# JKc66/CircuitVision

Measured on AMD Instinct MI355X. Metric: circuit images/sec (YOLOv11 640² + SAM2.1-L 1024²) at 1/2/4/8 MI355X, higher is better.
Workload: dtype f16; 1 GPU; YOLO11-n 640x640 batch=32 f16 forward+decode+NMS (BASELINE configs[1]) + SAM2.1 Hiera-L 1024x1024 2 x batch=16 f16 learned-prompt wrapper forward (configs[2]) on the same images, per GPU and step; nc=62, weights=seeded random (SAM: LoRA merged), streams=3

## Files before the change

circuitvision_amd/_lib.py:

```python
import ctypes as C
import os

_HERE = os.path.dirname(os.path.abspath(__file__))
LIB_PATH = os.environ.get("CVMI_LIB_PATH") or os.path.join(_HERE, "libcvmi355.so")

F16, F32, BF16 = 0, 1, 2
ACT_NONE, ACT_SILU, ACT_RELU, ACT_GELU, ACT_SIGMOID = 0, 1, 2, 3, 4


class CvmiError(RuntimeError):
    pass


class ConvDesc(C.Structure):
    _fields_ = [
        ("x0", C.c_void_p), ("x1", C.c_void_p), ("w", C.c_void_p), ("bias", C.c_void_p),
        ("res", C.c_void_p), ("y", C.c_void_p),
        ("x0_ld", C.c_int), ("x1_ld", C.c_int), ("res_ld", C.c_int), ("y_ld", C.c_int),
        ("c0", C.c_int), ("c1", C.c_int), ("up0", C.c_int), ("up1", C.c_int),
        ("B", C.c_int), ("H", C.c_int), ("W", C.c_int), ("OH", C.c_int), ("OW", C.c_int),
        ("KH", C.c_int), ("KW", C.c_int), ("stride", C.c_int), ("pad", C.c_int),
        ("N", C.c_int), ("Kpad", C.c_int), ("act", C.c_int), ("dtype", C.c_int),
        ("out_f32", C.c_int), ("scalar_gather", C.c_int),
        ("res_mod", C.c_int), ("act_after_res", C.c_int), ("shuffle_cout", C.c_int), ("res_rep", C.c_int),
        ("row_stats", C.c_void_p),
    ]


class C3k2Desc(C.Structure):
    _fields_ = [
        ("x", C.c_void_p), ("y", C.c_void_p),
        ("w0", C.c_void_p), ("w1", C.c_void_p), ("w2", C.c_void_p), ("w3", C.c_void_p),
        ("b0", C.c_void_p), ("b1", C.c_void_p), ("b2", C.c_void_p), ("b3", C.c_void_p),
        ("x_ld", C.c_int), ("y_ld", C.c_int), ("kpad0", C.c_int), ("kpad1", C.c_int), ("kpad2", C.c_int), ("kpad3", C.c_int),
        ("B", C.c_int), ("H", C.c_int), ("W", C.c_int), ("c1", C.c_int), ("c", C.c_int), ("h", C.c_int), ("c2", C.c_int),
        ("fuse_cv1", C.c_int), ("shortcut", C.c_int), ("dtype", C.c_int),
    ]


class DwPwDesc(C.Structure):
    _fields_ = [
        ("x", C.c_void_p), ("y", C.c_void_p), ("wd", C.c_void_p), ("bd", C.c_void_p),
        ("w1", C.c_void_p), ("b1", C.c_void_p), ("w2", C.c_void_p), ("b2", C.c_void_p),
        ("x_ld", C.c_int), ("y_ld", C.c_int), ("kpad1", C.c_int), ("kpad2", C.c_int),
        ("B", C.c_int), ("H", C.c_int), ("W", C.c_int), ("C", C.c_int), ("N1", C.c_int), ("N2", C.c_int),
        ("dtype", C.c_int),
    ]


class AttnDesc(C.Structure):
    _fields_ = [
        ("q", C.c_void_p), ("k", C.c_void_p), ("v", C.c_void_p), ("o", C.c_void_p),
        ("q_sb", C.c_longlong), ("q_sh", C.c_longlong), ("q_st", C.c_longlong),
        ("k_sb", C.c_longlong), ("k_sh", C.c_longlong), ("k_st", C.c_longlong),
        ("v_sb", C.c_longlong), ("v_sh", C.c_longlong), ("v_st", C.c_longlong),
        ("o_sb", C.c_longlong), ("o_sh", C.c_longlong), ("o_st", C.c_longlong),
        ("B", C.c_int), ("heads", C.c_int), ("Nq", C.c_int), ("Nk", C.c_int),
        ("dqk", C.c_int), ("dv", C.c_int), ("scale", C.c_float), ("dtype", C.c_int),
# ... 142 lines not shown
```

circuitvision_amd/csrc/igemm.hip:

```cpp
#include "conv_epilogue.hpp"

namespace {

struct ConvKArgs {
  const char* x0; const char* x1; const char* w; const float* bias; const char* res; char* y;
  int x0_ld, x1_ld, res_ld, y_ld;
  int c0, ctot;
  int up0, up1;
  int H, W, OH, OW, KW, stride, pad;
  int M, N, K, Kpad;
  int act, scalar_gather;
  int res_mod, act_after_res, shuf_c, res_rep;
  int plain;
  int rows2;
  int nb_n;
  int bias_off;
  int per_xcd;
  float* stats;
  int im2col_shift;
  FastDiv div_ctot, div_kw;
};

__device__ __attribute__((aligned(256))) unsigned char cvmi_zero_page[256];

__device__ __forceinline__ int xcd_remap(int wg, int nwg) {
  const int q = nwg >> 3, r = nwg & 7, xcd = wg & 7, j = wg >> 3;
  return (xcd < r ? xcd * (q + 1) : r * (q + 1) + (xcd - r) * q) + j;
}

#define CLEAR_ACC32(acc, NI, NJ) \
  _Pragma("unroll") for (int i = 0; i < NI; ++i) \
  _Pragma("unroll") for (int j = 0; j < NJ; ++j) \
  _Pragma("unroll") for (int r = 0; r < 16; ++r) acc[i][j][r] = 0.f
// ... 1335 lines not shown
  constexpr int glds_min_tiles = 512;
  if ((a.plain || a.rows2) && a.K % (16 / (int)sizeof(T)) == 0 && (a.Kpad * (int)sizeof(T)) % 128 == 0 && a.K * (int)sizeof(T) >= 256 &&
      ((a.K * (int)sizeof(T)) % 128 == 0 || a.K >= 256) && N >= (a.rows2 ? 64 : 96) &&
      (long long)cdiv(M, 128) * cdiv(N, 128) >= glds_min_tiles) {
    if (N <= 640) return launch_glds<T, TO, 128, 64, 2, 2>(a, stream);
    return launch_glds<T, TO, 128, 128, 2, 2>(a, stream);
  }
  if (N <= 32) {
    if (M >= 256 * 512) return launch_cfg<T, TO, 256, 32, 4, 1>(a, stream);
    return launch_cfg<T, TO, 128, 32, 4, 1>(a, stream);
  }
  if (N <= 64) {
    if (M >= 128 * 512) return launch_cfg<T, TO, 128, 64, 2, 2>(a, stream);
    return launch_cfg<T, TO, 64, 64, 2, 2>(a, stream);
  }
  if (sizeof(TO) == 4 && sizeof(T) == 2 && N <= 192) return launch_cfg<T, TO, 128, 64, 2, 2>(a, stream);
  const long long blocks128 = (long long)cdiv(M, 128) * cdiv(N, 128);
  if (blocks128 >= 512) return launch_cfg<T, TO, 128, 128, 2, 2>(a, stream);
  return launch_cfg<T, TO, 64, 128, 2, 2>(a, stream);
}

}

int cvmi_conv_tile_try(const cvmi_conv_desc* d, hipStream_t stream);
#ifndef CVMI_OPERAND_BF16
extern "C" int cvmi_conv2d_bf16(const cvmi_conv_desc* d, cvmi_stream_t stream_);
#endif

extern "C" int CVMI_ENTRY(cvmi_conv2d)(const cvmi_conv_desc* d, cvmi_stream_t stream_) {
  CVMI_CHECK(d != nullptr, "conv2d: null descriptor");
#ifndef CVMI_OPERAND_BF16
  if (d->dtype == CVMI_BF16) return cvmi_conv2d_bf16(d, stream_);
#endif
  CVMI_CHECK(d->x0 && d->w && d->bias && d->y, "conv2d: null pointer");
  CVMI_CHECK(d->dtype == CVMI_T16 || d->dtype == CVMI_F32, "conv2d: bad dtype %d", d->dtype);
  const int es = d->dtype == CVMI_T16 ? 2 : 4;
  const int vec = 16 / es;
  const int oes = (d->dtype == CVMI_F32 || d->out_f32) ? 4 : 2;
  const int ovec = 16 / oes;
  CVMI_CHECK(d->B > 0 && d->H > 0 && d->W > 0 && d->OH > 0 && d->OW > 0 && d->N > 0, "conv2d: bad shape");
  CVMI_CHECK(d->KH > 0 && d->KW > 0 && d->stride > 0 && d->pad >= 0, "conv2d: bad kernel geometry");
  CVMI_CHECK(d->c0 > 0 && d->c1 >= 0 && (d->c1 == 0 || d->x1), "conv2d: bad sources");
  CVMI_CHECK((d->OH - 1) * d->stride - d->pad + d->KH - 1 < d->H + d->pad &&
             (d->OW - 1) * d->stride - d->pad + d->KW - 1 < d->W + d->pad, "conv2d: output larger than input allows");
  const int ctot = d->c0 + d->c1;
  const long long K = (long long)d->KH * d->KW * ctot;
  CVMI_CHECK(K < 65536 && d->Kpad >= K && d->Kpad % 32 == 0 && d->Kpad <= 65536, "conv2d: K=%lld Kpad=%d unsupported", K, d->Kpad);
  if (!d->scalar_gather) {
    CVMI_CHECK(d->c0 % vec == 0 && d->c1 % vec == 0, "conv2d: channels (%d,%d) not multiples of %d", d->c0, d->c1, vec);
    CVMI_CHECK(d->x0_ld % vec == 0 && (d->c1 == 0 || d->x1_ld % vec == 0), "conv2d: source ld not 16-byte aligned");
    CVMI_CHECK(((uintptr_t)d->x0 & 15) == 0 && ((uintptr_t)d->x1 & 15) == 0, "conv2d: source not 16-byte aligned");
  }
  CVMI_CHECK(d->x0_ld >= d->c0 && (d->c1 == 0 || d->x1_ld >= d->c1), "conv2d: ld smaller than channels");
  CVMI_CHECK(d->y_ld % ovec == 0 && ((uintptr_t)d->y & 15) == 0, "conv2d: output not 16-byte aligned");
  CVMI_CHECK(d->y_ld >= d->N || d->shuffle_cout > 0, "conv2d: y_ld < N");
  CVMI_CHECK(!d->res || (d->res_ld % ovec == 0 && ((uintptr_t)d->res & 15) == 0 && (d->res_ld >= d->N || d->shuffle_cout > 0)), "conv2d: residual misaligned");
  CVMI_CHECK(((uintptr_t)d->w & 15) == 0 && ((uintptr_t)d->bias & 15) == 0, "conv2d: weights misaligned");
  CVMI_CHECK(d->up0 == 0 || (d->H % 2 == 0 && d->W % 2 == 0), "conv2d: upsampled source needs even H, W");
  CVMI_CHECK(d->up1 == 0 || (d->H % 2 == 0 && d->W % 2 == 0), "conv2d: upsampled source needs even H, W");
  const long long M = (long long)d->B * d->OH * d->OW;
  CVMI_CHECK(M < (1ll << 31), "conv2d: M too large");

  ConvKArgs a;
  a.x0 = (const char*)d->x0; a.x1 = (const char*)d->x1; a.w = (const char*)d->w; a.bias = d->bias;
  a.res = (const char*)d->res; a.y = (char*)d->y;
  a.x0_ld = d->x0_ld; a.x1_ld = d->x1_ld; a.res_ld = d->res_ld; a.y_ld = d->y_ld;
// ... 36 lines not shown
```

circuitvision_amd/engine.py:

```python
import ctypes as C
import os
import threading

import torch

from . import _lib
from ._lib import BF16, F16, F32, AttnDesc, C3k2Desc, ConvDesc

TORCH_DTYPE = {F16: torch.float16, F32: torch.float32, BF16: torch.bfloat16}
ESIZE = {F16: 2, F32: 4, BF16: 2}
DTYPE_OF = {torch.float16: F16, torch.float32: F32, torch.bfloat16: BF16}


def is16(dtype):
    return dtype in (F16, BF16)


def require_gpu():
    if not torch.cuda.is_available():
        raise _lib.CvmiError("circuitvision_amd needs an MI355X (gfx950) GPU: torch.cuda.is_available() is False; "
                             "there is no CPU fallback")
    _lib.load()


# ... 525 lines not shown
        return dict(wp=wp[:C_].clone(), bp=bias[:C_].clone(), w1=w1, b1=f1[:, C_] + f1[:, C_ + 1], w2=f2[:C_].clone(), b2=bias[C_:].clone())


def op_hiera_mlp(plan, label, pm, x, gamma, beta, eps=1e-6, stats_out=None, stats_eps=1e-6, proj=None):
    lib = _lib.load()
    if proj is not None:
        pm, ao = proj[0], _as_rows(proj[1])
    assert x.dtype == F32 and x.c == pm.C and x.c0 == 0
    rows = x.B * x.H * x.W
    assert stats_out is None or (stats_out.dtype == torch.float32 and stats_out.numel() == 2 * rows and stats_out.is_contiguous()), label
    desc, b2 = None, pm.bias.data_ptr()
    if proj is not None:
        assert ao.rows == rows and ao.C == pm.C and ao.dtype == pm.dtype, label
        desc = _lib.MlpProj(ao=ao.ptr, w_packed=pm.w.data_ptr(), bp=pm.bias.data_ptr(), ao_ld=ao.ld)
        b2 += 4 * pm.C
    args = (x.ptr, x.ld, gamma.data_ptr(), beta.data_ptr(), float(eps), None if proj is not None else pm.w.data_ptr(), b2, rows, pm.C, pm.dtype,
            stats_out.data_ptr() if stats_out is not None else None, float(stats_eps))
    plan.keep.append((pm, x, gamma, beta, stats_out, proj, desc))
    sp0, fn = plan.sptr, lib.cvmi_hiera_mlp_stats
    pdesc = C.byref(desc) if desc is not None else None

    def thunk(sp=None):
        sp = sp0 if sp is None else sp
        _lib.check(fn(*args, sp, pdesc), label)

    plan.add(label, "mlp_fused", thunk, rows * pm.C * (8 + (ESIZE[pm.dtype] if proj is not None else 0)),
             2 * rows * 2 * 4 * pm.C * pm.C + (2 * rows * pm.C * pm.C if proj is not None else 0))


def tok_linear_supported(K, dtype, rows):
    return is16(dtype) and rows % 256 == 0 and bool(_lib.load().cvmi_tok_linear_supported(K))


class PackedTokLinear:

    def __init__(self, w, b, device="cuda", dtype=F16):
        N, K = w.shape
        td = TORCH_DTYPE[dtype]
        assert K % 16 == 0
        if _lib.load().cvmi_tok_linear_format(K) == 16:
            nch, ks = (N + 31) // 32, K // 32
            b = b if b is not None else torch.zeros(N)
            wx = torch.zeros(nch * 32, K)
            wx[:N] = w
            frag = wx.view(nch, 2, 16, ks, 4, 8).permute(0, 3, 1, 4, 2, 5).reshape(nch, ks * 2 * 512)
            bias = torch.zeros(nch * 32)
            bias[:N] = b
            piece = torch.zeros(nch, 512, dtype=torch.int16)
            piece[:, :64] = bias.view(nch, 32).contiguous().view(torch.int16)
            packed = torch.cat((frag.to(td).contiguous().view(torch.int16), piece), 1).contiguous()
            assert packed.numel() * 2 == _lib.load().cvmi_tok_linear_packed_bytes(K, N)
            self.w = packed.to(device)
            self.bias = torch.zeros(4, device=device)
            self.N, self.K, self.dtype = N, K, dtype
            self.param_bytes = N * K * 2
            return
        ks1, nch = K // 16 + 1, ((N + 31) // 32 + 1) // 2 * 2
        b = b if b is not None else torch.zeros(N)
        b_hi = b.to(td).float()
        b_lo = (b - b_hi).to(td).float()
        wx = torch.zeros(nch * 32, K + 16)
        wx[:N, :K], wx[:N, K], wx[:N, K + 1] = w, b_hi, b_lo
        packed = wx.view(nch, 32, ks1, 2, 8).permute(0, 2, 3, 1, 4).contiguous()
        assert packed.numel() * 2 == _lib.load().cvmi_tok_linear_packed_bytes(K, N)
        self.w = packed.to(td).to(device)
        self.bias = torch.zeros(4, device=device)
        self.N, self.K, self.dtype = N, K, dtype
        self.param_bytes = N * K * 2


def qkv_attn_rows(heads, hd=72):
    C_ = heads * hd
    rows = []
    for h in range(heads):
        for c in range(3):
            for r in range(32):
                g, lh, e = r >> 3, (r >> 2) & 1, r & 3
                d = 32 * c + 16 * (g >> 1) + 8 * lh + 4 * (g & 1) + e
                rows.append(h * hd + d if d < hd else -1)
        rows += [C_ + h * hd + n if n < hd else 2 * C_ + h * hd + n - hd if n < 2 * hd else -1 for n in range(160)]
    return rows


def qkv_attn_supported(dim, dout, heads, ws, q_pool, dtype, nwin):
    return is16(dtype) and dim == 144 and ws == 8 and nwin % 2 == 0 and (dout, heads) == ((288, 4) if q_pool else (144, 2))


def qkv_attn16_supported(dim, dout, heads, ws, q_pool, dtype, nwin):
    return is16(dtype) and dim == 288 and ws == 4 and nwin % 8 == 0 and (dout, heads) == ((576, 8) if q_pool else (288, 4))


class PackedQkvAttn:

    def __init__(self, w, b, heads, device="cuda", dtype=F16):
        N, K = w.shape
        assert N % (3 * heads) == 0
        self.rows = qkv_attn_rows(heads, N // (3 * heads))
        idx = torch.tensor(self.rows)
        keep = (idx >= 0).float()
        b = b if b is not None else torch.zeros(N)
        pt = PackedTokLinear(w[idx.clamp(min=0)] * keep[:, None], b[idx.clamp(min=0)] * keep, device, dtype)
        self.w, self.bias = pt.w, pt.bias
        self.N, self.K, self.heads, self.dtype = N, K, heads, dtype
        self.param_bytes = pt.param_bytes


def tok_linear_stats_parts(rows, K, N):
    return int(_lib.load().cvmi_tok_linear_stats_parts(rows, K, N))


def op_tok_linear(plan, label, pt, src, dst, ln=None, act=_lib.ACT_NONE, residual=False, kind="gemm", stats_in=None, stats_out=None, stats_eps=1e-6,
                  stats_parts=0):
    lib = _lib.load()
    src, dst = _as_rows(src), _as_rows(dst)
    assert src.C == pt.K and dst.C == pt.N and src.rows == dst.rows and src.rows % 256 == 0, label
    assert (src.dtype == F32) == (ln is not None) and (dst.dtype == F32) == bool(residual), label
    assert (ln is not None or src.dtype == pt.dtype) and (residual or dst.dtype == pt.dtype), label
    cast = isinstance(ln, str)
    assert not cast or ln == "cast", label
    assert stats_in is None or (ln is not None and not cast), label
    assert stats_out is None or residual, label
    out_parts = tok_linear_stats_parts(src.rows, pt.K, pt.N) if stats_out is not None else 0
    assert stats_out is None or (stats_out.dtype == torch.float32 and stats_out.numel() == 2 * src.rows * max(out_parts, 1) and stats_out.is_contiguous()), label
    assert stats_in is None or (stats_in.dtype == torch.float32 and stats_in.numel() == 2 * src.rows * max(stats_parts, 1) and stats_in.is_contiguous()), label
    gam, bet, eps = ln if (ln is not None and not cast) else (None, None, 0.0)
    args = (src.ptr, src.ld, 2 if cast else 1 if ln is not None else 0, gam.data_ptr() if gam is not None else None, bet.data_ptr() if bet is not None else None,
            float(eps), pt.w.data_ptr(), dst.ptr, dst.ld, 1 if residual else 0, src.rows, pt.K, pt.N, act, pt.dtype,
            stats_in.data_ptr() if stats_in is not None else None, int(stats_parts), stats_out.data_ptr() if stats_out is not None else None, float(stats_eps))
    plan.keep.append((pt, src, dst, gam, bet, stats_in, stats_out))
    sp0, fn = plan.sptr, lib.cvmi_tok_linear_stats

    def thunk(sp=None):
        sp = sp0 if sp is None else sp
        _lib.check(fn(*args, sp), label)

    bytes_ = src.rows * (pt.K * ESIZE[src.dtype] + pt.N * ESIZE[dst.dtype] * (2 if residual else 1))
    plan.add(label, kind, thunk, bytes_, 2 * src.rows * pt.N * pt.K)


# ... 19 lines not shown
```

circuitvision_amd/sam2.py:

```python
import hashlib
import math
import os
import threading

import numpy as np
import torch
import torch.nn.functional as TF

from . import _lib
from ._lib import ACT_GELU, ACT_NONE, ACT_RELU, ACT_SIGMOID, BF16, F16, F32
from .engine import (ESIZE, TORCH_DTYPE, is16, Buf, PackedConv, PackedHieraMlp, PackedProjMlp, PackedQkvAttn, PackedTokLinear, Plan, Rows, hiera_mlp_supported, make_attn_desc, op_attention,
                     op_call, op_cast, op_conv, op_hiera_mlp, op_layernorm, op_maxpool2, op_tok_linear, op_tok_linear_pool, require_gpu, row_stats_supported,
                     qkv_attn16_supported, qkv_attn_supported, tok_linear_stats_parts, tok_linear_supported)

LOG2E = 1.4426950408889634
HIERA_L = dict(embed_dim=144, num_heads=2, stages=(2, 6, 36, 4), global_att_blocks=(23, 33, 43), window_spec=(8, 4, 16, 8))
HIERA_T = dict(embed_dim=96, num_heads=1, stages=(1, 2, 7, 2), global_att_blocks=(5, 7, 9), window_spec=(8, 4, 14, 7))

LORA_TARGETS_REFERENCE = (
    [f"sam_mask_decoder.transformer.layers.{l}.{a}.{p}" for l in (0, 1) for a in ("self_attn", "cross_attn_token_to_image")
     for p in ("k_proj", "q_proj", "v_proj", "out_proj")]
    + [f"sam_mask_decoder.transformer.layers.{l}.mlp.layers.{j}" for l in (0, 1) for j in (0, 1)]
    + ["sam_mask_decoder.iou_prediction_head.layers.2", "sam_mask_decoder.conv_s0", "sam_mask_decoder.conv_s1",
       "image_encoder.neck.convs.2.conv", "image_encoder.neck.convs.3.conv",
       "image_encoder.trunk.blocks.44.attn.qkv", "image_encoder.trunk.blocks.44.mlp.layers.0", "image_encoder.trunk.blocks.44.proj",
       "image_encoder.trunk.blocks.47.attn.qkv", "image_encoder.trunk.blocks.47.mlp.layers.0"]
    + [f"sam_mask_decoder.transformer.layers.{l}.cross_attn_image_to_token.{p}" for l in (0, 1) for p in ("q_proj", "k_proj", "v_proj")])


MASK_DOWN = "sam_prompt_encoder.mask_downscaling"
MASK_DOWN_PARAMS = 4684


def mask_down_tensors():
    return [(f"{MASK_DOWN}.0.weight", (4, 1, 2, 2), "w"), (f"{MASK_DOWN}.0.bias", (4,), "w"),
            (f"{MASK_DOWN}.1.weight", (4,), "gamma"), (f"{MASK_DOWN}.1.bias", (4,), "w"),
            (f"{MASK_DOWN}.3.weight", (16, 4, 2, 2), "w"), (f"{MASK_DOWN}.3.bias", (16,), "w"),
            (f"{MASK_DOWN}.4.weight", (16,), "gamma"), (f"{MASK_DOWN}.4.bias", (16,), "w"),
            (f"{MASK_DOWN}.6.weight", (256, 16, 1, 1), "w"), (f"{MASK_DOWN}.6.bias", (256,), "w")]


class SamSyntheticParams:

    def __init__(self, seed=0, lora_targets=LORA_TARGETS_REFERENCE, r=4, alpha=16, std=0.02):
        self.seed, self.targets, self.r, self.scaling, self.std, self.sd = seed, set(lora_targets), r, alpha / r, std, {}
        self.mask_sd = {}
# ... 140 lines not shown
        self.pc[key] = pc
        self.param_bytes += pc.param_bytes
        return pc

    def _linear(self, key, mod, cout, cin, tok=False, row_scale=None, fuse_heads=0):
        w, b = self.p.weight(mod, (cout, cin)), self.p.bias(mod, cout)
        if row_scale is not None:
            n, f = row_scale
            w, b = w.clone(), b.clone()
            w[:n] *= f
            b[:n] *= f
        if tok and self.use_tok and is16(self.dtype) and tok_linear_supported(cin, self.dtype, 256):
            self.tl[key] = PackedTokLinear(w, b, self.device, self.dtype)
            if fuse_heads:
                self.tl[key + "_attn"] = PackedQkvAttn(w, b, fuse_heads, self.device, self.dtype)
        return self._pack(key, _lin(w), b)

    def _norm(self, key, mod, c):
        self.ln[key] = (self.p.tensor(f"{mod}.weight", (c,), "gamma").float().to(self.device),
                        self.p.tensor(f"{mod}.bias", (c,)).float().to(self.device))

    def _trunk(self):
        h = self.hiera
        E, stages, ws = h["embed_dim"], h["stages"], h["window_spec"]
        T = "image_encoder.trunk"
        w7 = self.p.weight(f"{T}.patch_embed.proj", (E, 3, 7, 7))
        w2 = torch.zeros(E, 48, 2, 2)
        m = {k: ((0, k + 1) if k < 3 else (1, k - 3)) for k in range(7)}
        for ky in range(7):
            for kx in range(7):
                (ty, sy), (tx, sx) = m[ky], m[kx]
                w2[:, (sy * 4 + sx) * 3:(sy * 4 + sx) * 3 + 3, ty, tx] = w7[:, :, ky, kx]
        self._pack("patch_embed", w2, self.p.bias(f"{T}.patch_embed.proj", E))
        g = self.image_size // 4
        pos = TF.interpolate(self.p.tensor(f"{T}.pos_embed", (1, E, 7, 7)), size=(g, g), mode="bicubic")
        win = self.p.tensor(f"{T}.pos_embed_window", (1, E, ws[0], ws[0]))
        pos = pos + win.tile([1, 1, g // ws[0], g // ws[0]])
        self.const["pos_embed"] = pos.permute(0, 2, 3, 1).reshape(g * g, E).contiguous().float().to(self.device)
        stage_ends = [sum(stages[:i]) - 1 for i in range(1, len(stages) + 1)]
        q_pool_blocks = [x + 1 for x in stage_ends[:-1]][:3]
        self.blocks, self.stage_ends = [], stage_ends
        cur, dim, heads = 1, E, h["num_heads"]
        for i in range(sum(stages)):
            dim_out, window = dim, ws[cur - 1]
            if i in h["global_att_blocks"]:
                window = 0
            if i - 1 in stage_ends:
                dim_out, heads, cur = dim * 2, heads * 2, cur + 1
            b = f"{T}.blocks.{i}"
            self._norm(f"b{i}.norm1", f"{b}.norm1", dim)
            self._linear(f"b{i}.qkv", f"{b}.attn.qkv", 3 * dim_out, dim, tok=True,
                         row_scale=(dim_out, (dim_out // heads) ** -0.5 * LOG2E) if self.q_log2 else None,
                         fuse_heads=heads if (self.qkv_attn and qkv_attn_supported(dim, dim_out, heads, window, i in q_pool_blocks, self.dtype, 2))
                         or (self.qkv_attn16 and qkv_attn16_supported(dim, dim_out, heads, window, i in q_pool_blocks, self.dtype, 8)) else 0)
            self._linear(f"b{i}.proj", f"{b}.attn.proj", dim_out, dim_out, tok=True)
            self._norm(f"b{i}.norm2", f"{b}.norm2", dim_out)
            if self.fused_mlp and hiera_mlp_supported(dim_out, self.dtype):
                self.mlp[f"b{i}"] = PackedHieraMlp(self.p.weight(f"{b}.mlp.layers.0", (4 * dim_out, dim_out)), self.p.bias(f"{b}.mlp.layers.0", 4 * dim_out),
                                                   self.p.weight(f"{b}.mlp.layers.1", (dim_out, 4 * dim_out)), self.p.bias(f"{b}.mlp.layers.1", dim_out),
                                                   self.device, self.dtype)
                self.param_bytes += self.mlp[f"b{i}"].param_bytes
                self.mlp[f"b{i}.projmlp"] = PackedProjMlp(self.p.weight(f"{b}.attn.proj", (dim_out, dim_out)), self.p.bias(f"{b}.attn.proj", dim_out),
                                                          self.p.weight(f"{b}.mlp.layers.0", (4 * dim_out, dim_out)), self.p.bias(f"{b}.mlp.layers.0", 4 * dim_out),
                                                          self.p.weight(f"{b}.mlp.layers.1", (dim_out, 4 * dim_out)), self.p.bias(f"{b}.mlp.layers.1", dim_out),
                                                          self.device, self.dtype)
            else:
# ... 167 lines not shown
        self.mask_prompt, self.multimask = bool(mask_prompt), bool(multimask)
        self.plan = Plan(stream)
        self.pool = {}
        self.dynamic = dynamic_multimask_via_stability
        self.act_bytes = 0
        self._build()
        torch.cuda.synchronize()

    def buf(self, H, W, C, dtype=None, tag=None, zero=False, batch=None):
        dtype = self.dt if dtype is None else dtype
        batch = self.B if batch is None else batch
        key = (batch, H, W, C, dtype, tag)
        if tag is None or key not in self.pool:
            b = Buf(batch, H, W, C, dtype, self.dev, zero=zero)
            self.act_bytes += b.nbytes
            if tag is None:
                return b
            self.pool[key] = b
        return self.pool[key]

    def gemm(self, label, key, src, dst, act=ACT_NONE, res=None, kind="gemm", **kw):
        srcs = src if isinstance(src, list) else [(src, 0)]
        op_conv(self.plan, label, self.wt.pc[key], srcs, dst, act=act, res=res, kind=kind, **kw)

    def _build(self):
        wt, B = self.wt, self.B
        R = wt.image_size
        g = R // 4
        self.x_in = Buf(B, R, R, 3, self.dt, self.dev, zero=True)
        E = wt.hiera["embed_dim"]
        x = self.buf(g, g, E, F32)
        pos = wt.const["pos_embed"]
        self.plan.keep.append(pos)
        xs = Buf(B, g, g, 48, self.dt, self.dev)
        lib = _lib.load()
        op_call(self.plan, "s2d4", "stem", lib.cvmi_space_to_depth4, (self.x_in.t.data_ptr(), xs.t.data_ptr(), B, R, R, self.dt),
                keep=(self.x_in, xs), bytes_=2 * self.x_in.nbytes)
        op_conv(self.plan, "patch_embed", wt.pc["patch_embed"], [(xs.view(), 0)], x.view(), stride=1, pad=1, out_hw=(g, g),
                res=_ConstView(pos, E), res_mod=g * g, kind="stem")
        H = W = g
        stage_out = []
        for i, blk in enumerate(wt.blocks):
            x, H, W = self._block(i, blk, x, H, W)
            if i in wt.stage_ends:
                stage_out.append(x)
        self.stage_out = stage_out
        self._neck_decoder(stage_out)

    def _block(self, i, blk, x, H, W):
        wt, B = self.wt, self.B
        dim, dout, heads, ws = blk["dim"], blk["dim_out"], blk["heads"], blk["window"]
        hd = dout // heads
        gam, bet = wt.ln[f"b{i}.norm1"]
        Hp, Wp = (H, W) if ws == 0 else (-(-H // ws) * ws, -(-W // ws) * ws)
        padded = (Hp, Wp) != (H, W)
        if blk["q_pool"] and (ws == 0 or ws % 2 or Hp % 2 or Wp % 2):
            raise NotImplementedError("q-pool block needs an even window")
        tok_rows = not padded and (B * H * W) % 256 == 0
        tok_qkv = tok_rows and f"b{i}.qkv" in wt.tl
        if dim != dout and os.environ.get("CVMI_SAM_QKVTOK_TRANS", "1") == "0":
            tok_qkv = False
        tok_pool = tok_rows and dim != dout and f"b{i}.dimproj" in wt.tl and os.environ.get("CVMI_SAM_POOLFUSE", "1") != "0"
        if padded:
            xn = self.buf(Hp, Wp, dim, tag="xn_padded", zero=True)
            op_layernorm(self.plan, f"b{i}.norm1", x.view(), gam, bet, xn.view(), 1e-6, pad=(H, W, Hp, Wp))
        elif not tok_qkv or (dim != dout and not tok_pool):
            xn = self.buf(H, W, dim, tag="xn")
            op_layernorm(self.plan, f"b{i}.norm1", x.view(), gam, bet, xn.view(), 1e-6)
        parts = self._ln1_parts
        ln1_stats = self._ln1_stats if (self._ln1_stats is not None and self._ln1_stats.numel() == 2 * B * H * W * max(parts, 1)) else None
        self._ln1_stats, self._ln1_parts = None, 0
        if dim != dout:
# ... 311 lines not shown
```

include/cvmi355.h:

```cpp
#ifndef CVMI355_H
#define CVMI355_H

#include <stddef.h>
#include <stdint.h>

#ifdef __cplusplus
extern "C" {
#endif

#define CVMI_VERSION 127

typedef void* cvmi_stream_t;

enum { CVMI_F16 = 0, CVMI_F32 = 1, CVMI_BF16 = 2 };
enum { CVMI_ACT_NONE = 0, CVMI_ACT_SILU = 1, CVMI_ACT_RELU = 2, CVMI_ACT_GELU = 3, CVMI_ACT_SIGMOID = 4 };

int cvmi_version(void);
const char* cvmi_last_error(void);
const char* cvmi_last_kernel(void);
int cvmi_device_info(int device, int* out4);
enum { CVMI_DESC_CONV = 0, CVMI_DESC_C3K2 = 1, CVMI_DESC_DWPW = 2, CVMI_DESC_ATTN = 3 };
size_t cvmi_desc_size(int kind);

int cvmi_graph_begin(cvmi_stream_t stream);
int cvmi_graph_end(cvmi_stream_t stream, void** graph_exec_out);
int cvmi_graph_launch(void* graph_exec, cvmi_stream_t stream);
int cvmi_graph_destroy(void* graph_exec);

typedef struct cvmi_conv_desc {
  const void* x0; const void* x1;
  const void* w; const float* bias;
  const void* res;
  void* y;
  int x0_ld, x1_ld, res_ld, y_ld;
  int c0, c1;
  int up0, up1;
  int B, H, W;
  int OH, OW;
  int KH, KW, stride, pad;
  int N;
  int Kpad;
  int act;
  int dtype;
  int out_f32;
  int scalar_gather;
  int res_mod;
  int act_after_res;
  int shuffle_cout;
  int res_rep;
  float* row_stats;
} cvmi_conv_desc;
int cvmi_conv2d(const cvmi_conv_desc* d, cvmi_stream_t stream);

typedef struct {
  const void* x; void* y;
  const void *w0, *w1, *w2, *w3;
  const float *b0, *b1, *b2, *b3;
  int x_ld, y_ld, kpad0, kpad1, kpad2, kpad3;
  int B, H, W, c1, c, h, c2;
  int fuse_cv1, shortcut, dtype;
} cvmi_c3k2_desc;
int cvmi_c3k2_supported(int c1, int c, int h, int c2, int fuse_cv1, int dtype);
int cvmi_c3k2(const cvmi_c3k2_desc* d, cvmi_stream_t stream);

int cvmi_stem2_supported(int c0, int c1, int dtype);
int cvmi_stem2(const void* x, int x_ld, const void* w0, const float* b0, int kpad0, const void* w1, const float* b1, int kpad1,
               void* y, int y_ld, int B, int H2, int W2, int c0, int c1, int dtype, cvmi_stream_t stream);

typedef struct {
  const void* x; void* y;
  const void* wd; const float* bd;
  const void* w1; const float* b1;
  const void* w2; const float* b2;
  int x_ld, y_ld, kpad1, kpad2;
  int B, H, W, C, N1, N2;
  int dtype;
} cvmi_dwpw_desc;
int cvmi_dwpw_supported(int C, int N1, int N2, int dtype);
int cvmi_dwpw(const cvmi_dwpw_desc* d, cvmi_stream_t stream);

int cvmi_dwconv3x3(const void* x, int x_ld, const void* w, const float* bias, const void* res,
                   int res_ld, void* y, int y_ld, int B, int H, int W, int C, int act, int dtype,
                   cvmi_stream_t stream);
// ... 222 lines not shown
```

Measured before the change: 412.9 images/s.

## Fuse SAM patch-embed space-to-depth, conv, pos-add and LN stats into one kernel

Adds a dedicated MFMA patch-embed kernel that reads the raw image directly with a reordered 192-wide K layout, which removes the separate space-to-depth pass and its intermediate buffer. The same kernel adds the positional table and, when possible, emits per-row mean/rstd for block 0's layernorm so that stats pass can be skipped. The goal is to cut a full-image round trip plus one stats read of the 256x256x144 f32 activation. It brings in a specialised kernel with hard-coded geometry and edge masking logic, and it only applies for E=144 with 16-bit dtypes.

```diff
diff --git a/circuitvision_amd/_lib.py b/circuitvision_amd/_lib.py
--- a/circuitvision_amd/_lib.py
+++ b/circuitvision_amd/_lib.py
@@ -24,6 +24,7 @@
         ("out_f32", C.c_int), ("scalar_gather", C.c_int),
         ("res_mod", C.c_int), ("act_after_res", C.c_int), ("shuffle_cout", C.c_int), ("res_rep", C.c_int),
         ("row_stats", C.c_void_p),
+        ("patch_image", C.c_void_p), ("stats_out", C.c_void_p), ("stats_eps", C.c_float),
     ]
 
 
diff --git a/circuitvision_amd/csrc/igemm.hip b/circuitvision_amd/csrc/igemm.hip
--- a/circuitvision_amd/csrc/igemm.hip
+++ b/circuitvision_amd/csrc/igemm.hip
@@ -1,4 +1,5 @@
 #include "conv_epilogue.hpp"
+#include "patch_embed.hpp"
 
 namespace {
 
@@ -1400,6 +1401,8 @@
 #ifndef CVMI_OPERAND_BF16
   if (d->dtype == CVMI_BF16) return cvmi_conv2d_bf16(d, stream_);
 #endif
+  if (d->patch_image) return launch_patch_embed(d, (hipStream_t)stream_);
+  CVMI_CHECK(!d->stats_out, "conv2d: stats_out belongs to the patch_image form");
   CVMI_CHECK(d->x0 && d->w && d->bias && d->y, "conv2d: null pointer");
   CVMI_CHECK(d->dtype == CVMI_T16 || d->dtype == CVMI_F32, "conv2d: bad dtype %d", d->dtype);
   const int es = d->dtype == CVMI_T16 ? 2 : 4;
diff --git a/circuitvision_amd/csrc/patch_embed.hpp b/circuitvision_amd/csrc/patch_embed.hpp
--- /dev/null
+++ b/circuitvision_amd/csrc/patch_embed.hpp
@@ -0,0 +1,192 @@
+#pragma once
+#include "tok_stream.hpp"
+
+namespace {
+
+constexpr int PE_N = 144, PE_K = 192, PE_KS = PE_K / 32, PE_NF = 2 * PE_KS;
+constexpr int PE_NCH = (PE_N + 31) / 32, PE_CHB = (PE_NF + 1) * 1024;
+constexpr int PE_LDS = PE_NCH * PE_CHB;
+constexpr int PE_NW = 8, PE_TILE = PE_NW * 32;
+constexpr int PE_NQ = PE_N / 16;
+
+struct PatchArgs {
+  const f16* img;
+  const char* wp;
+  const float* pos;
+  float* out;
+  float* stats;
+  long long rows;
+  int H, W, gh, gw, out_ld, pos_ld;
+  float eps;
+  int njobs, B, tpi, ppx;
+};
+
+typedef u32x4 pe_u32x4_a8 __attribute__((aligned(8)));
+
+struct PeTile {
+  u32x4 xn[2][PE_KS];
+  unsigned zm[2], hm[2];
+  const float* pr[2];
+  long long row[2];
+};
+
+template <typename T>
+__global__ __launch_bounds__(PE_NW * 64, 2) void patch_embed_kernel(const PatchArgs a) {
+  static_assert(sizeof(T) == 2, "16-bit operands");
+  extern __shared__ __attribute__((aligned(16))) char smem[];
+  const int tid = threadIdx.x, wv = __builtin_amdgcn_readfirstlane(tid >> 6), lane = tid & 63;
+  const int c16 = lane & 15, g = lane >> 4;
+  tok_issue_chunk<PE_NCH * (PE_NF + 1), PE_NW>(a.wp, smem, wv, lane);
+
+  int off[PE_KS];
+  unsigned pc0 = 0, pc1 = 0;
+#pragma unroll
+  for (int s = 0; s < PE_KS; ++s) {
+    const int p = 4 * s + g, wy = p / 3, pc = p - 3 * wy;
+    off[s] = wy * a.W * 3 + 8 * pc;
+    pc0 |= (pc == 0 ? 1u : 0u) << s;
+    pc1 |= (pc == 1 ? 1u : 0u) << s;
+  }
+  const unsigned gg = (unsigned)(a.gh * a.gw);
+  const bool stats = a.stats != nullptr;
+
+  auto tile_of = [&](int job) -> long long {
+    if (a.ppx == 0) return job;
+    const int k = job >> 3, pl = k / a.B;
+    return (long long)(k - pl * a.B) * a.tpi + (job & 7) * a.ppx + pl;
+  };
+  auto load_tile = [&](int job, PeTile& t) {
+    const long long wrow0 = tile_of(job) * PE_TILE + wv * 32;
+#pragma unroll
+    for (int tg = 0; tg < 2; ++tg) {
+      const long long r = wrow0 + 16 * tg + c16;
+      t.row[tg] = r < a.rows ? r : -1;
+      const unsigned tk = (unsigned)(r < a.rows ? r : a.rows - 1);
+      const unsigned b = tk / gg, prow = tk - b * gg;
+      const unsigned oy = prow / (unsigned)a.gw, ox = prow - oy * (unsigned)a.gw;
+      const bool top = oy == 0, left = ox == 0;
+      const f16* const wbase = a.img + (((long long)b * a.H + 4 * (long long)oy - 4) * a.W + 4 * (long long)ox - 4) * 3;
+      t.zm[tg] = (top ? 7u : 0u) | (left ? pc0 : 0u);
+      t.hm[tg] = left ? pc1 : 0u;
+#pragma unroll
+      for (int s = 0; s < PE_KS; ++s) {
+        const f16* p = wbase + off[s] + (s < 3 && top ? 4 * a.W * 3 : 0) + (left ? (((pc0 >> s) & 1u) ? 12 : ((pc1 >> s) & 1u) ? 4 : 0) : 0);
+        t.xn[tg][s] = *reinterpret_cast<const pe_u32x4_a8*>(p);
+      }
+      t.pr[tg] = a.pos + (size_t)prow * a.pos_ld + 4 * g;
+    }
+  };
+  auto fix_tile = [&](PeTile& t) {
+#pragma unroll
+    for (int tg = 0; tg < 2; ++tg)
+#pragma unroll
+      for (int s = 0; s < PE_KS; ++s) {
+        const bool zero = (t.zm[tg] >> s) & 1u, half = (t.hm[tg] >> s) & 1u;
+        const u32x4 ld = t.xn[tg][s];
+        u32x4 v;
+        v[0] = zero || half ? 0u : ld[0];
+        v[1] = zero || half ? 0u : ld[1];
+        v[2] = zero ? 0u : half ? ld[0] : ld[2];
+        v[3] = zero ? 0u : half ? ld[1] : ld[3];
+        t.xn[tg][s] = v;
+      }
+  };
+
+  asm volatile("s_waitcnt vmcnt(0)" ::: "memory");
+  tok_barrier();
+
+  int job = blockIdx.x;
+  if (job >= a.njobs) return;
+  PeTile t;
+  load_tile(job, t);
+#pragma unroll 1
+  for (;;) {
+    fix_tile(t);
+    f32x4 acc[2][PE_NQ];
+#pragma unroll
+    for (int q = 0; q < PE_NQ; ++q) {
+      const char* const buf = smem + (q >> 1) * PE_CHB;
+      acc[0][q] = acc[1][q] = *reinterpret_cast<const f32x4*>(buf + PE_NF * 1024 + (q & 1) * 64 + g * 16);
+#pragma unroll
+      for (int s = 0; s < PE_KS; ++s) {
+        const f16x8 w8 = *reinterpret_cast<const f16x8*>(buf + (2 * s + (q & 1)) * 1024 + lane * 16);
+        acc[0][q] = CVMI_MFMA_16X16X32(w8, __builtin_bit_cast(f16x8, t.xn[0][s]), acc[0][q], 0, 0, 0);
+        acc[1][q] = CVMI_MFMA_16X16X32(w8, __builtin_bit_cast(f16x8, t.xn[1][s]), acc[1][q], 0, 0, 0);
+      }
+      __builtin_amdgcn_sched_barrier(0);
+    }
+    const long long row[2] = {t.row[0], t.row[1]};
+    {
+      f32x4 pv[2][PE_NQ];
+#pragma unroll
+      for (int tg = 0; tg < 2; ++tg)
+#pragma unroll
+        for (int q = 0; q < PE_NQ; ++q) pv[tg][q] = *reinterpret_cast<const f32x4*>(t.pr[tg] + 16 * q);
+#pragma unroll
+      for (int tg = 0; tg < 2; ++tg)
+#pragma unroll
+        for (int q = 0; q < PE_NQ; ++q) acc[tg][q] += pv[tg][q];
+    }
+    float2 mr[2];
+    if (stats) {
+#pragma unroll
+      for (int tg = 0; tg < 2; ++tg) {
+        ShiftedSums st;
+        st.shift = __shfl(acc[tg][0][0], c16);
+#pragma unroll
+        for (int q = 0; q < PE_NQ; ++q) st.add(acc[tg][q]);
+        mr[tg] = shifted_mean_rstd(st.shift, row_sum<4>(st.s), row_sum<4>(st.q), (float)PE_N, a.eps);
+      }
+    }
+    job += gridDim.x;
+    const bool more = job < a.njobs;
+    if (more) load_tile(job, t);
+    __builtin_amdgcn_sched_barrier(0);
+#pragma unroll
+    for (int tg = 0; tg < 2; ++tg) {
+      if (row[tg] >= 0) {
+        float* const op = a.out + (size_t)row[tg] * a.out_ld + 4 * g;
+#pragma unroll
+        for (int q = 0; q < PE_NQ; ++q) *reinterpret_cast<f32x4*>(op + 16 * q) = acc[tg][q];
+        if (stats && g == 0) *reinterpret_cast<float2*>(a.stats + 2 * row[tg]) = mr[tg];
+      }
+    }
+    if (!more) break;
+  }
+}
+
+int launch_patch_embed(const cvmi_conv_desc* d, hipStream_t stream) {
+  CVMI_CHECK(d->dtype == CVMI_T16, "patch_embed: dtype %d is not built (fp16 / bf16 only)", d->dtype);
+  CVMI_CHECK(d->N == PE_N, "patch_embed: Cout=%d is not built (144 only)", d->N);
+  CVMI_CHECK(d->B > 0 && d->H > 0 && d->W > 0 && d->H % 4 == 0 && d->W % 4 == 0, "patch_embed: image %d x %d x %d: sides must be positive multiples of 4", d->B, d->H, d->W);
+  CVMI_CHECK(d->OH == d->H / 4 && d->OW == d->W / 4 && d->KH == 7 && d->KW == 7 && d->stride == 4 && d->pad == 3 && d->c0 == 3 && d->c1 == 0,
+             "patch_embed: geometry must be 3 channels, 7 x 7, stride 4, pad 3, output H/4 x W/4");
+  CVMI_CHECK(d->w && d->res && d->y && d->out_f32 && d->res_mod == d->OH * d->OW && d->act == CVMI_ACT_NONE && !d->act_after_res && d->shuffle_cout == 0 &&
+             d->res_rep <= 1 && !d->row_stats, "patch_embed: needs the packed weight, f32 output and the positional table as res with res_mod = OH * OW");
+  CVMI_CHECK(((uintptr_t)d->patch_image & 7) == 0 && ((uintptr_t)d->w & 15) == 0 && ((uintptr_t)d->res & 15) == 0 && ((uintptr_t)d->y & 15) == 0 &&
+             ((uintptr_t)d->stats_out & 7) == 0 && d->y_ld % 4 == 0 && d->res_ld % 4 == 0 && d->y_ld >= PE_N && d->res_ld >= PE_N,
+             "patch_embed: misaligned pointer or row stride (image 8 bytes, weight / table / output 16, statistics 8)");
+  const long long rows = (long long)d->B * d->OH * d->OW;
+  CVMI_CHECK(rows < (1ll << 31) && (long long)d->B * d->H * d->W * 3 < (1ll << 40), "patch_embed: %lld tokens: too many", rows);
+  static hipError_t attr = hipFuncSetAttribute(reinterpret_cast<const void*>(&patch_embed_kernel<f16>), hipFuncAttributeMaxDynamicSharedMemorySize, PE_LDS);
+  CVMI_HIP(attr);
+  static const int ncu = [] {
+    int dev = 0;
+    hipDeviceProp_t prop;
+    if (hipGetDevice(&dev) != hipSuccess || hipGetDeviceProperties(&prop, dev) != hipSuccess) return 256;
+    return prop.multiProcessorCount > 0 ? prop.multiProcessorCount : 256;
+  }();
+  const int gg = d->OH * d->OW;
+  const bool by_position = d->B > 1 && gg % (8 * PE_TILE) == 0;
+  const int tpi = by_position ? gg / PE_TILE : 0, ppx = tpi / 8;
+  const long long njobs = (rows + PE_TILE - 1) / PE_TILE;
+  const unsigned grid = (unsigned)(njobs < ncu ? njobs : ncu);
+  const PatchArgs a{(const f16*)d->patch_image, (const char*)d->w, (const float*)d->res, (float*)d->y, d->stats_out, rows,
+                    d->H, d->W, d->OH, d->OW, d->y_ld, d->res_ld, d->stats_eps, (int)njobs, d->B, tpi, ppx};
+  cvmi_note_kernel("patch_embed_kernel<%s>", CVMI_F16NAME);
+  hipLaunchKernelGGL((patch_embed_kernel<f16>), dim3(grid), dim3(PE_NW * 64), PE_LDS, stream, a);
+  CVMI_LAUNCH_CHECK();
+  return 0;
+}
+
+}
diff --git a/circuitvision_amd/engine.py b/circuitvision_amd/engine.py
--- a/circuitvision_amd/engine.py
+++ b/circuitvision_amd/engine.py
@@ -581,6 +581,30 @@
     return is16(dtype) and rows % 256 == 0 and bool(_lib.load().cvmi_tok_linear_supported(K))
 
 
+def _pack_tok16(w, b, td):
+    N, K = w.shape
+    nch, ks = (N + 31) // 32, K // 32
+    b = b if b is not None else torch.zeros(N)
+    wx = torch.zeros(nch * 32, K)
+    wx[:N] = w
+    frag = wx.view(nch, 2, 16, ks, 4, 8).permute(0, 3, 1, 4, 2, 5).reshape(nch, ks * 2 * 512)
+    bias = torch.zeros(nch * 32)
+    bias[:N] = b
+    piece = torch.zeros(nch, 512, dtype=torch.int16)
+    piece[:, :64] = bias.view(nch, 32).contiguous().view(torch.int16)
+    return torch.cat((frag.to(td).contiguous().view(torch.int16), piece), 1).contiguous()
+
+
+def _unpack_tok16(packed, N, K, td):
+    nch, ks = (N + 31) // 32, K // 32
+    packed = packed.cpu().view(nch, -1)
+    w = packed[:, :ks * 1024].contiguous().view(td).float().view(nch, ks, 2, 4, 16, 8).permute(0, 2, 4, 1, 3, 5).reshape(nch * 32, K)
+    piece = packed[:, ks * 1024:]
+    bias = piece[:, :64].contiguous().view(torch.float32).reshape(nch * 32)
+    assert not w[N:].any() and not bias[N:].any() and not piece[:, 64:].any()
+    return w[:N].clone(), bias[:N].clone()
+
+
 class PackedTokLinear:
 
     def __init__(self, w, b, device="cuda", dtype=F16):
@@ -588,16 +612,7 @@
         td = TORCH_DTYPE[dtype]
         assert K % 16 == 0
         if _lib.load().cvmi_tok_linear_format(K) == 16:
-            nch, ks = (N + 31) // 32, K // 32
-            b = b if b is not None else torch.zeros(N)
-            wx = torch.zeros(nch * 32, K)
-            wx[:N] = w
-            frag = wx.view(nch, 2, 16, ks, 4, 8).permute(0, 3, 1, 4, 2, 5).reshape(nch, ks * 2 * 512)
-            bias = torch.zeros(nch * 32)
-            bias[:N] = b
-            piece = torch.zeros(nch, 512, dtype=torch.int16)
-            piece[:, :64] = bias.view(nch, 32).contiguous().view(torch.int16)
-            packed = torch.cat((frag.to(td).contiguous().view(torch.int16), piece), 1).contiguous()
+            packed = _pack_tok16(w, b, td)
             assert packed.numel() * 2 == _lib.load().cvmi_tok_linear_packed_bytes(K, N)
             self.w = packed.to(device)
             self.bias = torch.zeros(4, device=device)
@@ -654,6 +669,65 @@
         self.param_bytes = pt.param_bytes
 
 
+PATCH_EMBED_K = 192
+
+
+def patch_embed_k_order():
+    out = []
+    for k in range(PATCH_EMBED_K):
+        wy, wx, c = k // 24, (k % 24) // 3, k % 3
+        out.append((c * 7 + wy - 1) * 7 + wx - 1 if wy and wx else -1)
+    return out
+
+
+def patch_embed_supported(E, R, dtype):
+    return is16(dtype) and E == 144 and R > 0 and R % 4 == 0
+
+
+class PackedPatchEmbed:
+
+    def __init__(self, w7, bias, device="cuda", dtype=F16):
+        E = w7.shape[0]
+        assert tuple(w7.shape) == (E, 3, 7, 7)
+        idx = torch.tensor(patch_embed_k_order())
+        w = w7.reshape(E, 147).float()[:, idx.clamp(min=0)] * (idx >= 0).float()[None]
+        self.w = _pack_tok16(w, bias.float() if bias is not None else None, TORCH_DTYPE[dtype]).to(device)
+        self.bias = torch.zeros(4, device=device)
+        self.N, self.K, self.dtype = E, PATCH_EMBED_K, dtype
+        self.param_bytes = E * 147 * 2
+
+    def unpack(self):
+        w, b = _unpack_tok16(self.w, self.N, self.K, TORCH_DTYPE[self.dtype])
+        idx = torch.tensor(patch_embed_k_order())
+        assert not w[:, idx < 0].any()
+        w7 = torch.zeros(self.N, 147)
+        w7[:, idx[idx >= 0]] = w[:, idx >= 0]
+        return w7.view(self.N, 3, 7, 7), b
+
+
+def op_patch_embed(plan, label, pp, img, dst, pos, stats_out=None, stats_eps=1e-6, kind="stem"):
+    lib = _lib.load()
+    B, H, W = img.B, img.H, img.W
+    OH, OW = H // 4, W // 4
+    assert img.C == 3 and img.dtype == pp.dtype and dst.dtype == F32 and (dst.B, dst.H, dst.W, dst.c) == (B, OH, OW, pp.N), label
+    assert pos.dtype == torch.float32 and tuple(pos.shape) == (OH * OW, pp.N) and pos.is_contiguous(), label
+    rows = B * OH * OW
+    assert stats_out is None or (stats_out.dtype == torch.float32 and stats_out.numel() == 2 * rows and stats_out.is_contiguous()), label
+    d = ConvDesc(w=pp.w.data_ptr(), res=pos.data_ptr(), y=dst.ptr, res_ld=pp.N, y_ld=dst.ld, c0=3, B=B, H=H, W=W, OH=OH, OW=OW, KH=7, KW=7,
+                 stride=4, pad=3, N=pp.N, dtype=pp.dtype, out_f32=1, res_mod=OH * OW, patch_image=img.t.data_ptr(),
+                 stats_out=(stats_out.data_ptr() if stats_out is not None else None), stats_eps=float(stats_eps))
+    plan.keep.append((d, pp, img, dst, pos, stats_out))
+    sp0, fn = plan.sptr, lib.cvmi_conv2d
+
+    def thunk(sp=None):
+        sp = sp0 if sp is None else sp
+        _lib.check(fn(C.byref(d), sp), label)
+
+    bytes_ = img.nbytes + rows * pp.N * 4 + OH * OW * pp.N * 4 + pp.w.numel() * 2
+    plan.add(label, kind, thunk, bytes_, 2 * rows * 147 * pp.N)
+    return d
+
+
 def tok_linear_stats_parts(rows, K, N):
     return int(_lib.load().cvmi_tok_linear_stats_parts(rows, K, N))
 
diff --git a/circuitvision_amd/sam2.py b/circuitvision_amd/sam2.py
--- a/circuitvision_amd/sam2.py
+++ b/circuitvision_amd/sam2.py
@@ -11,7 +11,8 @@
 from ._lib import ACT_GELU, ACT_NONE, ACT_RELU, ACT_SIGMOID, BF16, F16, F32
 from .engine import (ESIZE, TORCH_DTYPE, is16, Buf, PackedConv, PackedHieraMlp, PackedProjMlp, PackedQkvAttn, PackedTokLinear, Plan, Rows, hiera_mlp_supported, make_attn_desc, op_attention,
                      op_call, op_cast, op_conv, op_hiera_mlp, op_layernorm, op_maxpool2, op_tok_linear, op_tok_linear_pool, require_gpu, row_stats_supported,
-                     qkv_attn16_supported, qkv_attn_supported, tok_linear_stats_parts, tok_linear_supported)
+                     qkv_attn16_supported, qkv_attn_supported, tok_linear_stats_parts, tok_linear_supported,
+                     PackedPatchEmbed, op_patch_embed, patch_embed_supported)
 
 LOG2E = 1.4426950408889634
 HIERA_L = dict(embed_dim=144, num_heads=2, stages=(2, 6, 36, 4), global_att_blocks=(23, 33, 43), window_spec=(8, 4, 16, 8))
@@ -218,6 +219,8 @@
                 (ty, sy), (tx, sx) = m[ky], m[kx]
                 w2[:, (sy * 4 + sx) * 3:(sy * 4 + sx) * 3 + 3, ty, tx] = w7[:, :, ky, kx]
         self._pack("patch_embed", w2, self.p.bias(f"{T}.patch_embed.proj", E))
+        if patch_embed_supported(E, self.image_size, self.dtype):
+            self.tl["patch_embed"] = PackedPatchEmbed(w7, self.p.bias(f"{T}.patch_embed.proj", E), self.device, self.dtype)
         g = self.image_size // 4
         pos = TF.interpolate(self.p.tensor(f"{T}.pos_embed", (1, E, 7, 7)), size=(g, g), mode="bicubic")
         win = self.p.tensor(f"{T}.pos_embed_window", (1, E, ws[0], ws[0]))
@@ -451,12 +454,20 @@
         x = self.buf(g, g, E, F32)
         pos = wt.const["pos_embed"]
         self.plan.keep.append(pos)
-        xs = Buf(B, g, g, 48, self.dt, self.dev)
         lib = _lib.load()
-        op_call(self.plan, "s2d4", "stem", lib.cvmi_space_to_depth4, (self.x_in.t.data_ptr(), xs.t.data_ptr(), B, R, R, self.dt),
-                keep=(self.x_in, xs), bytes_=2 * self.x_in.nbytes)
-        op_conv(self.plan, "patch_embed", wt.pc["patch_embed"], [(xs.view(), 0)], x.view(), stride=1, pad=1, out_hw=(g, g),
-                res=_ConstView(pos, E), res_mod=g * g, kind="stem")
+        if "patch_embed" in wt.tl and os.environ.get("CVMI_SAM_PATCHEMBED", "1") != "0":
+            ws0 = wt.blocks[0]["window"]
+            b0_stats = ("b0.qkv" in wt.tl and (B * g * g) % 256 == 0 and (ws0 == 0 or g % ws0 == 0)
+                        and os.environ.get("CVMI_SAM_LNSTATS", "1") != "0")
+            stats = torch.empty(B * g * g, 2, dtype=torch.float32, device=self.dev) if b0_stats else None
+            op_patch_embed(self.plan, "patch_embed", wt.tl["patch_embed"], self.x_in, x.view(), pos, stats_out=stats, stats_eps=1e-6)
+            self._ln1_stats, self._ln1_parts = stats, 0
+        else:
+            xs = Buf(B, g, g, 48, self.dt, self.dev)
+            op_call(self.plan, "s2d4", "stem", lib.cvmi_space_to_depth4, (self.x_in.t.data_ptr(), xs.t.data_ptr(), B, R, R, self.dt),
+                    keep=(self.x_in, xs), bytes_=2 * self.x_in.nbytes)
+            op_conv(self.plan, "patch_embed", wt.pc["patch_embed"], [(xs.view(), 0)], x.view(), stride=1, pad=1, out_hw=(g, g),
+                    res=_ConstView(pos, E), res_mod=g * g, kind="stem")
         H = W = g
         stage_out = []
         for i, blk in enumerate(wt.blocks):
diff --git a/include/cvmi355.h b/include/cvmi355.h
--- a/include/cvmi355.h
+++ b/include/cvmi355.h
@@ -8,7 +8,7 @@
 extern "C" {
 #endif
 
-#define CVMI_VERSION 127
+#define CVMI_VERSION 128
 
 typedef void* cvmi_stream_t;
 
@@ -49,6 +49,9 @@
   int shuffle_cout;
   int res_rep;
   float* row_stats;
+  const void* patch_image;
+  float* stats_out;
+  float stats_eps;
 } cvmi_conv_desc;
 int cvmi_conv2d(const cvmi_conv_desc* d, cvmi_stream_t stream);
 
```

Measured after the change: 415.5 images/s, median of 6. No clear change (+0.6%).
